# robot-learning-freiburg/CL-SLAM

Hardware: AMD Instinct MI355X
Metric: online-adapt frames/sec @192x640 (1 triplet + K replay) (higher is better)
Workload: dtype f32; 1 GPU; DepthPosePrediction.adapt(steps=1), 192x640, 1 online + K=4 replay triplets (global batch 5); ResNet-18 depth+pose nets, closed-form random-init weights; a frame = 5 triplets (value = steps/s * B/5); global_batch=5, replay_k=4, height=192, width=640, adapt_steps_per_frame=1, parallelism=single, lcd_encoder_in_frame=False

## Files before the change

### cl-slam_amd/csrc/wgrad_patch.hip

```cpp
#include "common.h"

namespace clslam {

struct WgPatchK {
    const float* __restrict__ dz;
    const float* __restrict__ src_a;
    const float* __restrict__ src_b;
    float* __restrict__ partial;
    int B, Hi, Wi, Ca, Cb, Ho, Wo, Cout;
    int pad, pad_mode, ups;
    int tilesX, tilesY, ntiles, tiles_per_split, co_tiles, ci_tiles;
};

template <int TH, int TW, int COT, int CIT>
__global__ __launch_bounds__(256) void conv3x3_wgrad_patch_kernel(WgPatchK p) {
    constexpr int BM = TH * TW;
    constexpr int PH = TH + 2, PW = TW + 2, PP = PH * PW;
    constexpr int LDZ = (COT % 32 == 16) ? COT : COT + 16;
    constexpr int LDP = (CIT % 32 == 16) ? CIT : CIT + 16;
    constexpr int TI = COT / 16, TJ = CIT / 16;
    constexpr int Z_F4 = BM * COT / 4, P_F4 = PP * CIT / 4;
    constexpr int Z_IT = (Z_F4 + 255) / 256, P_IT = (P_F4 + 255) / 256;

    constexpr int SMEM = (BM * LDZ + PP * LDP) > (4 * TI * TJ * 256) ? (BM * LDZ + PP * LDP) : (4 * TI * TJ * 256);
    __shared__ __attribute__((aligned(16))) float smem[SMEM];
    float* const Zs = smem;
    float* const Ps = smem + BM * LDZ;

    const int tid = threadIdx.x, lane = tid & 63, wave = tid >> 6;
    const int cot = blockIdx.x % p.co_tiles, cit = blockIdx.x / p.co_tiles;
    const int split = blockIdx.y;
    const int co0 = cot * COT, ci0 = cit * CIT;
    const int Cin = p.Ca + p.Cb;
    const int HA = p.ups ? (p.Hi >> 1) : p.Hi, WA = p.ups ? (p.Wi >> 1) : p.Wi;
    const bool fromA = ci0 < p.Ca;
    const int csrc = fromA ? ci0 : ci0 - p.Ca;
    const int Csrc = fromA ? p.Ca : p.Cb;

    static_assert(TW % 4 == 0, "a pixel quad must not straddle two tile rows");
    const float* __restrict__ src = fromA ? p.src_a : p.src_b;
    f32x4 acc[9][TI][TJ];
#pragma unroll
    for (int t = 0; t < 9; ++t)
#pragma unroll
        for (int i = 0; i < TI; ++i)
#pragma unroll
            for (int j = 0; j < TJ; ++j)
#pragma unroll
                for (int r = 0; r < 4; ++r) acc[t][i][j][r] = 0.f;

    const int l16 = lane & 15, kg = lane >> 4;
    const int t_beg = split * p.tiles_per_split;
    const int t_end = min(p.ntiles, t_beg + p.tiles_per_split);

    float4 rz[Z_IT], rp[P_IT];
    bool okz[Z_IT], okp[P_IT];
    auto load_tile = [&](int tile) {
        int q = tile;
        const int tx = q % p.tilesX; q /= p.tilesX;
        const int ty = q % p.tilesY; q /= p.tilesY;
        const int b = q;
        const int oy0 = ty * TH, ox0 = tx * TW;
#pragma unroll
        for (int it = 0; it < Z_IT; ++it) {
            const int f = tid + it * 256;
            const int m = f / (COT / 4), c4 = f % (COT / 4);
            const int oy = oy0 + m / TW, ox = ox0 + m % TW;
            const bool ok = (f < Z_F4) && oy < p.Ho && ox < p.Wo;
            const size_t o = ok ? (((size_t)b * p.Ho + oy) * p.Wo + ox) * p.Cout + co0 + c4 * 4 : 0;
            rz[it] = *reinterpret_cast<const float4*>(p.dz + o);
            okz[it] = ok;
        }
#pragma unroll
        for (int it = 0; it < P_IT; ++it) {
            const int f = tid + it * 256;
            const int pp = f / (CIT / 4), c4 = f % (CIT / 4);
            const int pr = pp / PW, pc = pp - pr * PW;
            int iy = oy0 - p.pad + pr, ix = ox0 - p.pad + pc;
            bool ok = f < P_F4;
            if (p.pad_mode == CLSLAM_PAD_REFLECT) {
                iy = reflect_idx(iy, p.Hi); ix = reflect_idx(ix, p.Wi);
                iy = min(max(iy, 0), p.Hi - 1); ix = min(max(ix, 0), p.Wi - 1);
            } else {
                ok = ok && iy >= 0 && iy < p.Hi && ix >= 0 && ix < p.Wi;
            }
            size_t o = 0;
            if (ok) {
                if (fromA) {
                    const int sy = p.ups ? (iy >> 1) : iy, sx = p.ups ? (ix >> 1) : ix;
                    o = ((size_t)(b * HA + sy) * WA + sx) * Csrc + csrc + c4 * 4;
                } else {
                    o = ((size_t)(b * p.Hi + iy) * p.Wi + ix) * Csrc + csrc + c4 * 4;
                }
            }
            rp[it] = *reinterpret_cast<const float4*>(src + o);
            okp[it] = ok;
        }
    };
    auto store_tile = [&]() {
#pragma unroll
        for (int it = 0; it < Z_IT; ++it) {
            const int f = tid + it * 256;
            float4 v = rz[it];
            if (!okz[it]) v = make_float4(0.f, 0.f, 0.f, 0.f);
            if (f < Z_F4) *reinterpret_cast<float4*>(&Zs[(f / (COT / 4)) * LDZ + (f % (COT / 4)) * 4]) = v;
        }
#pragma unroll
        for (int it = 0; it < P_IT; ++it) {
            const int f = tid + it * 256;
            float4 v = rp[it];
            if (!okp[it]) v = make_float4(0.f, 0.f, 0.f, 0.f);
            if (f < P_F4) *reinterpret_cast<float4*>(&Ps[(f / (CIT / 4)) * LDP + (f % (CIT / 4)) * 4]) = v;
        }
    };

    if (t_beg < t_end) load_tile(t_beg);
    for (int tile = t_beg; tile < t_end; ++tile) {
        __syncthreads();
        store_tile();
        __syncthreads();
        if (tile + 1 < t_end) load_tile(tile + 1);
#pragma unroll 2
        for (int ks = wave; ks < BM / 4; ks += 4) {
            const int pix = ks * 4 + kg;
            const int prow = (pix / TW) * PW + (pix % TW);
            float a[TI];
#pragma unroll
            for (int i = 0; i < TI; ++i) a[i] = Zs[pix * LDZ + i * 16 + l16];
#pragma unroll
            for (int tap = 0; tap < 9; ++tap) {
                const int off = (tap / 3) * PW + (tap % 3);
#pragma unroll
                for (int j = 0; j < TJ; ++j) {
                    const float bv = Ps[(prow + off) * LDP + j * 16 + l16];
#pragma unroll
                    for (int i = 0; i < TI; ++i) acc[tap][i][j] = mfma_16x16x4(a[i], bv, acc[tap][i][j]);
                }
            }
        }
    }

    float* out = p.partial + (size_t)split * p.Cout * 9 * Cin;
    float* red = smem;
#pragma unroll
    for (int tap = 0; tap < 9; ++tap) {
        __syncthreads();
#pragma unroll
        for (int i = 0; i < TI; ++i)
#pragma unroll
            for (int j = 0; j < TJ; ++j)
                *reinterpret_cast<f32x4*>(&red[((wave * TI * TJ + i * TJ + j) * 64 + lane) * 4]) = acc[tap][i][j];
        __syncthreads();
        for (int e = tid; e < TI * TJ * 64; e += 256) {
            const int ij = e / 64, ln = e % 64;
            f32x4 s4 = *reinterpret_cast<const f32x4*>(&red[(ij * 64 + ln) * 4]);
#pragma unroll
            for (int w = 1; w < 4; ++w) {
                const f32x4 v = *reinterpret_cast<const f32x4*>(&red[((w * TI * TJ + ij) * 64 + ln) * 4]);
                s4 += v;
            }
            const int i = ij / TJ, j = ij % TJ;
            const int ci = ci0 + j * 16 + (ln & 15);
#pragma unroll
            for (int r = 0; r < 4; ++r) {
                const int co = co0 + i * 16 + 4 * (ln >> 4) + r;
                out[((size_t)co * 9 + tap) * Cin + ci] = s4[r];
            }
        }
    }
}

template <int TH, int TW, int COT, int CIT>
static int launch_wgp(WgPatchK k, int splits, hipStream_t stream) {
    k.co_tiles = k.Cout / COT;
    k.ci_tiles = (k.Ca + k.Cb) / CIT;
    hipLaunchKernelGGL((conv3x3_wgrad_patch_kernel<TH, TW, COT, CIT>), dim3(k.co_tiles * k.ci_tiles, splits), dim3(256), 0,
                       stream, k);
    return check_launch("conv3x3_wgrad_patch");
}

static void wgp_tile(const clslam_conv_desc* d, int* cot, int* cit) {
    const int Cin = d->ch_a + d->ch_b;
    const bool c32 = d->ch_out % 32 == 0;
    const bool i32 = Cin % 32 == 0 && (d->ch_b == 0 || d->ch_a % 32 == 0);
    *cot = c32 ? 32 : 16;
    *cit = i32 ? 32 : 16;
    if (*cot == 32 && *cit == 16) *cot = 16;
}

static void wgp_pixel_tile(const clslam_conv_desc* d, int* th, int* tw) {
    int cot, cit;
    wgp_tile(d, &cot, &cit);
    *th = 8; *tw = 16;
    const char* env = getenv("CLSLAM_WGRAD_DEEP_TILES");
    const bool deep = env && atoi(env) != 0;
    if (cot == 32 && cit == 32 && deep) {
        if (d->out_w == 40 && d->out_h % 4 == 0) { *th = 4; *tw = 40; }
        else if (d->out_w == 20 && d->out_h == 6) { *th = 6; *tw = 20; }
    }
}

}

using namespace clslam;

extern "C" int clslam_wgrad_patch_supported(const clslam_conv_desc* d) {
    if (!(d->ksize == 3 && d->stride == 1 && d->out_h == d->in_h + 2 * d->pad - 2 && d->out_w == d->in_w + 2 * d->pad - 2 &&
          d->ch_out % 16 == 0 && (d->ch_a + d->ch_b) % 16 == 0 && d->ch_a % 16 == 0))
        return 0;
    if (d->out_w > 40) return 1;
    int th, tw;
    wgp_pixel_tile(d, &th, &tw);
    return th != 8;
}

extern "C" int clslam_wgrad_patch_splits(const clslam_conv_desc* d, int target_blocks) {
    int cot, cit, th, tw;
    wgp_tile(d, &cot, &cit);
    wgp_pixel_tile(d, &th, &tw);
    const int cols = (d->ch_out / cot) * ((d->ch_a + d->ch_b) / cit);
    const int ntiles = d->batch * cdiv(d->out_h, th) * cdiv(d->out_w, tw);
    const int splits = std::max(1, std::min(ntiles, cdiv(target_blocks, cols)));
    const int tps = cdiv(ntiles, splits);
    return cdiv(ntiles, tps);
}

extern "C" int clslam_conv_wgrad_patch(const clslam_conv_desc* d, const float* dz, float* partial, int splits, void* stream_) {
    hipStream_t stream = (hipStream_t)stream_;
    CLSLAM_REQUIRE(d && dz && partial && splits >= 1 && clslam_wgrad_patch_supported(d), "conv_wgrad_patch: unsupported conv");
    int cot, cit, th, tw;
    wgp_tile(d, &cot, &cit);
    wgp_pixel_tile(d, &th, &tw);
    WgPatchK k;
    k.dz = dz; k.src_a = d->src_a; k.src_b = d->src_b; k.partial = partial;
    k.B = d->batch; k.Hi = d->in_h; k.Wi = d->in_w; k.Ca = d->ch_a; k.Cb = d->ch_b; k.Ho = d->out_h; k.Wo = d->out_w;
    k.Cout = d->ch_out; k.pad = d->pad; k.pad_mode = d->pad_mode; k.ups = d->upsample_a;
    k.tilesX = cdiv(k.Wo, tw); k.tilesY = cdiv(k.Ho, th);
    k.ntiles = k.B * k.tilesX * k.tilesY;
    k.tiles_per_split = cdiv(k.ntiles, splits);
    k.co_tiles = k.ci_tiles = 0;
    if (th == 4) return launch_wgp<4, 40, 32, 32>(k, splits, stream);
    if (th == 6) return launch_wgp<6, 20, 32, 32>(k, splits, stream);
    if (cot == 32) return launch_wgp<8, 16, 32, 32>(k, splits, stream);
    if (cit == 32) return launch_wgp<8, 16, 16, 32>(k, splits, stream);
    return launch_wgp<8, 16, 16, 16>(k, splits, stream);
}
```

Before: 351.5 frames/s.

## Add parity-decomposed wgrad path for nearest-upsampled 3x3 convolution inputs

For decoder convs whose input is a 2x nearest-upsampled tensor with reflect padding, the weight gradient is computed on the low-resolution source. Output pixels are split into four parity classes, and each class correlates against a 2x2 neighbourhood instead of nine taps. The 9-tap weight gradient is then rebuilt by summing the class/offset accumulators, which cuts MFMA work and shrinks the patch tile staged in shared memory. The kernel also gains an amdgpu_waves_per_eu(2) hint. The parity path is on by default only for convs without a skip (ch_b) input and adds new index arithmetic that could be subtly wrong at reflect borders.

Result: no change. 353.1 frames/s (median of 6 runs) (+0.4%).

```diff
diff --git a/cl-slam_amd/csrc/wgrad_patch.hip b/cl-slam_amd/csrc/wgrad_patch.hip
--- a/cl-slam_amd/csrc/wgrad_patch.hip
+++ b/cl-slam_amd/csrc/wgrad_patch.hip
@@ -10,10 +10,151 @@
     int B, Hi, Wi, Ca, Cb, Ho, Wo, Cout;
     int pad, pad_mode, ups;
     int tilesX, tilesY, ntiles, tiles_per_split, co_tiles, ci_tiles;
+    int nine_blocks, nine_ci0;
 };
 
+constexpr int kParCIT = 16;
+
+template <int COT>
+__device__ __forceinline__ void wgp_parity_block(const WgPatchK& p, float* smem, int bx) {
+    constexpr int TH = 8, TW = 16, BM = TH * TW, CIT = kParCIT;
+    constexpr int QW = TW / 2, QP = BM / 4;
+    constexpr int PH = TH / 2 + 2, PW = TW / 2 + 2, PP = PH * PW;
+    constexpr int LDZ = (COT % 32 == 16) ? COT : COT + 16;
+    constexpr int LDP = CIT;
+    constexpr int TI = COT / 16;
+    constexpr int Z_F4 = BM * COT / 4, P_F4 = PP * CIT / 4;
+    constexpr int Z_IT = Z_F4 / 256;
+    static_assert(Z_F4 % 256 == 0 && P_F4 <= 256 && QP == 32, "staging loops below");
+    float* const Zs = smem;
+    float* const Ps = smem + BM * LDZ;
+
+    const int tid = threadIdx.x, lane = tid & 63, wave = tid >> 6;
+    const int cot = bx % p.co_tiles, cit = bx / p.co_tiles;
+    const int split = blockIdx.y;
+    const int co0 = cot * COT, ci0 = cit * CIT;
+    const int Cin = p.Ca + p.Cb;
+    const int HA = p.Hi >> 1, WA = p.Wi >> 1;
+
+    f32x4 acc[4][4][TI];
+#pragma unroll
+    for (int c = 0; c < 4; ++c)
+#pragma unroll
+        for (int s = 0; s < 4; ++s)
+#pragma unroll
+            for (int i = 0; i < TI; ++i)
+#pragma unroll
+                for (int r = 0; r < 4; ++r) acc[c][s][i][r] = 0.f;
+
+    const int l16 = lane & 15, kg = lane >> 4;
+    const int t_beg = split * p.tiles_per_split;
+    const int t_end = min(p.ntiles, t_beg + p.tiles_per_split);
+
+    float4 rz[Z_IT], rp;
+    bool okz[Z_IT];
+    auto load_tile = [&](int tile) {
+        int q = tile;
+        const int tx = q % p.tilesX; q /= p.tilesX;
+        const int ty = q % p.tilesY; q /= p.tilesY;
+        const int b = q;
+        const int oy0 = ty * TH, ox0 = tx * TW;
+#pragma unroll
+        for (int it = 0; it < Z_IT; ++it) {
+            const int f = tid + it * 256;
+            const int m = f / (COT / 4), c4 = f % (COT / 4);
+            const int oy = oy0 + m / TW, ox = ox0 + m % TW;
+            const bool ok = oy < p.Ho && ox < p.Wo;
+            const size_t o = ok ? (((size_t)b * p.Ho + oy) * p.Wo + ox) * p.Cout + co0 + c4 * 4 : 0;
+            rz[it] = *reinterpret_cast<const float4*>(p.dz + o);
+            okz[it] = ok;
+        }
+        {
+            const int f = tid < P_F4 ? tid : 0;
+            const int pp = f / (CIT / 4), c4 = f % (CIT / 4);
+            const int pr = pp / PW, pc = pp - pr * PW;
+            const int sy = min(max((oy0 >> 1) - 1 + pr, 0), HA - 1);
+            const int sx = min(max((ox0 >> 1) - 1 + pc, 0), WA - 1);
+            rp = *reinterpret_cast<const float4*>(p.src_a + ((size_t)(b * HA + sy) * WA + sx) * p.Ca + ci0 + c4 * 4);
+        }
+    };
+    auto store_tile = [&]() {
+#pragma unroll
+        for (int it = 0; it < Z_IT; ++it) {
+            const int f = tid + it * 256;
+            const int m = f / (COT / 4), c4 = f % (COT / 4);
+            const int my = m / TW, mx = m % TW;
+            const int row = ((my & 1) * 2 + (mx & 1)) * QP + (my >> 1) * QW + (mx >> 1);
+            float4 v = rz[it];
+            if (!okz[it]) v = make_float4(0.f, 0.f, 0.f, 0.f);
+            *reinterpret_cast<float4*>(&Zs[row * LDZ + c4 * 4]) = v;
+        }
+        if (tid < P_F4) *reinterpret_cast<float4*>(&Ps[(tid / (CIT / 4)) * LDP + (tid % (CIT / 4)) * 4]) = rp;
+    };
+
+    if (t_beg < t_end) load_tile(t_beg);
+    for (int tile = t_beg; tile < t_end; ++tile) {
+        __syncthreads();
+        store_tile();
+        __syncthreads();
+        if (tile + 1 < t_end) load_tile(tile + 1);
+#pragma unroll
+        for (int n = 0; n < 8; ++n) {
+            const int cls = n >> 1, py = cls >> 1, px = cls & 1;
+            const int q = ((n & 1) * 4 + wave) * 4 + kg;
+            const int prow = ((q / QW) + py) * PW + (q % QW) + px;
+            float a[TI];
+#pragma unroll
+            for (int i = 0; i < TI; ++i) a[i] = Zs[(cls * QP + q) * LDZ + i * 16 + l16];
+#pragma unroll
+            for (int s = 0; s < 4; ++s) {
+                const float bv = Ps[(prow + (s >> 1) * PW + (s & 1)) * LDP + l16];
+#pragma unroll
+                for (int i = 0; i < TI; ++i) acc[cls][s][i] = mfma_16x16x4(a[i], bv, acc[cls][s][i]);
+            }
+        }
+    }
+
+    float* out = p.partial + (size_t)split * p.Cout * 9 * Cin;
+    float* red = smem;
+#pragma unroll
+    for (int tap = 0; tap < 9; ++tap) {
+        const int ty = tap / 3, tx = tap % 3;
+        __syncthreads();
+#pragma unroll
+        for (int i = 0; i < TI; ++i) {
+            f32x4 s4 = acc[0][((ty + 1) >> 1) * 2 + ((tx + 1) >> 1)][i];
+            s4 += acc[1][((ty + 1) >> 1) * 2 + (tx >> 1)][i];
+            s4 += acc[2][(ty >> 1) * 2 + ((tx + 1) >> 1)][i];
+            s4 += acc[3][(ty >> 1) * 2 + (tx >> 1)][i];
+            *reinterpret_cast<f32x4*>(&red[((wave * TI + i) * 64 + lane) * 4]) = s4;
+        }
+        __syncthreads();
+        for (int e = tid; e < TI * 64; e += 256) {
+            const int i = e / 64, ln = e % 64;
+            f32x4 s4 = *reinterpret_cast<const f32x4*>(&red[(i * 64 + ln) * 4]);
+#pragma unroll
+            for (int w = 1; w < 4; ++w) {
+                const f32x4 v = *reinterpret_cast<const f32x4*>(&red[((w * TI + i) * 64 + ln) * 4]);
+                s4 += v;
+            }
+            const int ci = ci0 + (ln & 15);
+#pragma unroll
+            for (int r = 0; r < 4; ++r) {
+                const int co = co0 + i * 16 + 4 * (ln >> 4) + r;
+                out[((size_t)co * 9 + tap) * Cin + ci] = s4[r];
+            }
+        }
+    }
+}
+
+#if CLSLAM_DEVICE_BUILD
+#define WGP_TWO_WAVES __attribute__((amdgpu_waves_per_eu(2)))
+#else
+#define WGP_TWO_WAVES
+#endif
+
 template <int TH, int TW, int COT, int CIT>
-__global__ __launch_bounds__(256) void conv3x3_wgrad_patch_kernel(WgPatchK p) {
+__global__ __launch_bounds__(256) WGP_TWO_WAVES void conv3x3_wgrad_patch_kernel(WgPatchK p) {
     constexpr int BM = TH * TW;
     constexpr int PH = TH + 2, PW = TW + 2, PP = PH * PW;
     constexpr int LDZ = (COT % 32 == 16) ? COT : COT + 16;
@@ -27,10 +168,17 @@
     float* const Zs = smem;
     float* const Ps = smem + BM * LDZ;
 
+    if constexpr (TH == 8 && TW == 16) {
+        static_assert(SMEM >= BM * LDZ + (TH / 2 + 2) * (TW / 2 + 2) * kParCIT, "the parity form's tiles fit");
+        if ((int)blockIdx.x >= p.nine_blocks) {
+            wgp_parity_block<COT>(p, smem, (int)blockIdx.x - p.nine_blocks);
+            return;
+        }
+    }
     const int tid = threadIdx.x, lane = tid & 63, wave = tid >> 6;
     const int cot = blockIdx.x % p.co_tiles, cit = blockIdx.x / p.co_tiles;
     const int split = blockIdx.y;
-    const int co0 = cot * COT, ci0 = cit * CIT;
+    const int co0 = cot * COT, ci0 = p.nine_ci0 + cit * CIT;
     const int Cin = p.Ca + p.Cb;
     const int HA = p.ups ? (p.Hi >> 1) : p.Hi, WA = p.ups ? (p.Wi >> 1) : p.Wi;
     const bool fromA = ci0 < p.Ca;
@@ -171,10 +319,18 @@
 }
 
 template <int TH, int TW, int COT, int CIT>
-static int launch_wgp(WgPatchK k, int splits, hipStream_t stream) {
+static int launch_wgp(WgPatchK k, bool parity, int splits, hipStream_t stream) {
     k.co_tiles = k.Cout / COT;
     k.ci_tiles = (k.Ca + k.Cb) / CIT;
-    hipLaunchKernelGGL((conv3x3_wgrad_patch_kernel<TH, TW, COT, CIT>), dim3(k.co_tiles * k.ci_tiles, splits), dim3(256), 0,
+    k.nine_ci0 = 0;
+    k.nine_blocks = k.co_tiles * k.ci_tiles;
+    int blocks = k.nine_blocks;
+    if (parity && TH == 8 && TW == 16) {
+        k.nine_ci0 = k.Ca;
+        k.nine_blocks = k.co_tiles * (k.Cb / CIT);
+        blocks = k.nine_blocks + k.co_tiles * (k.Ca / kParCIT);
+    }
+    hipLaunchKernelGGL((conv3x3_wgrad_patch_kernel<TH, TW, COT, CIT>), dim3(blocks, splits), dim3(256), 0,
                        stream, k);
     return check_launch("conv3x3_wgrad_patch");
 }
@@ -200,14 +356,25 @@
     }
 }
 
+static bool wgp_parity(const clslam_conv_desc* d) {
+    const char* env = getenv("CLSLAM_WGRAD_PARITY");
+    const int mode = env ? atoi(env) : 1;
+    if (mode <= 0 || (mode == 1 && d->ch_b > 0)) return false;
+    return d->upsample_a && d->pad_mode == CLSLAM_PAD_REFLECT && d->pad == 1 && d->ch_a > 0 && d->in_h % 2 == 0 &&
+           d->in_w % 2 == 0 && d->in_h >= 2 && d->in_w >= 2;
+}
+
 }
 
 using namespace clslam;
 
+static bool wgp_valid(const clslam_conv_desc* d) {
+    return d->ksize == 3 && d->stride == 1 && d->out_h == d->in_h + 2 * d->pad - 2 && d->out_w == d->in_w + 2 * d->pad - 2 &&
+           d->ch_out % 16 == 0 && (d->ch_a + d->ch_b) % 16 == 0 && d->ch_a % 16 == 0;
+}
+
 extern "C" int clslam_wgrad_patch_supported(const clslam_conv_desc* d) {
-    if (!(d->ksize == 3 && d->stride == 1 && d->out_h == d->in_h + 2 * d->pad - 2 && d->out_w == d->in_w + 2 * d->pad - 2 &&
-          d->ch_out % 16 == 0 && (d->ch_a + d->ch_b) % 16 == 0 && d->ch_a % 16 == 0))
-        return 0;
+    if (!wgp_valid(d)) return 0;
     if (d->out_w > 40) return 1;
     int th, tw;
     wgp_pixel_tile(d, &th, &tw);
@@ -227,7 +394,7 @@
 
 extern "C" int clslam_conv_wgrad_patch(const clslam_conv_desc* d, const float* dz, float* partial, int splits, void* stream_) {
     hipStream_t stream = (hipStream_t)stream_;
-    CLSLAM_REQUIRE(d && dz && partial && splits >= 1 && clslam_wgrad_patch_supported(d), "conv_wgrad_patch: unsupported conv");
+    CLSLAM_REQUIRE(d && dz && partial && splits >= 1 && wgp_valid(d), "conv_wgrad_patch: unsupported conv");
     int cot, cit, th, tw;
     wgp_tile(d, &cot, &cit);
     wgp_pixel_tile(d, &th, &tw);
@@ -239,9 +406,10 @@
     k.ntiles = k.B * k.tilesX * k.tilesY;
     k.tiles_per_split = cdiv(k.ntiles, splits);
     k.co_tiles = k.ci_tiles = 0;
-    if (th == 4) return launch_wgp<4, 40, 32, 32>(k, splits, stream);
-    if (th == 6) return launch_wgp<6, 20, 32, 32>(k, splits, stream);
-    if (cot == 32) return launch_wgp<8, 16, 32, 32>(k, splits, stream);
-    if (cit == 32) return launch_wgp<8, 16, 16, 32>(k, splits, stream);
-    return launch_wgp<8, 16, 16, 16>(k, splits, stream);
-}
+    const bool par = wgp_parity(d);
+    if (th == 4) return launch_wgp<4, 40, 32, 32>(k, false, splits, stream);
+    if (th == 6) return launch_wgp<6, 20, 32, 32>(k, false, splits, stream);
+    if (cot == 32) return launch_wgp<8, 16, 32, 32>(k, par, splits, stream);
+    if (cit == 32) return launch_wgp<8, 16, 16, 32>(k, par, splits, stream);
+    return launch_wgp<8, 16, 16, 16>(k, par, splits, stream);
+}
```
